# HKUST-Aerial-Robotics/FUEL

Hardware: AMD Instinct MI355X
Metric: plan_cycles_per_sec (higher is better)
Workload: dtype u64 bit-planes / u16 (u32 beyond 255 voxels) exact squared distances / f32 ESDF / f64 log-odds and B-spline

## Files before the change

### fuel_amd/csrc/esdf.hip

```cpp
#include <algorithm>
#include <cmath>
#include <vector>

#include "fuelmi_internal.h"

template <int MODE>
__device__ __forceinline__ u64 src_word(const u64* __restrict__ infl, const u64* __restrict__ unk, long w) {
  if (MODE == 0) return infl[w] | unk[w];
  if (MODE == 1) return infl[w];
  return ~infl[w];
}

template <int MODE>
__device__ __forceinline__ int nearest_src(const u64* __restrict__ infl, const u64* __restrict__ unk,
                                           long linebit, int zlo, int zhi, int z) {
  int best = -1;
  {
    long pos = linebit + z, end = linebit + zhi;
    long w = pos >> 6;
    u64 word = src_word<MODE>(infl, unk, w) & (~0ull << (pos & 63));
    while (true) {
      if (word) {
        long c = (w << 6) + __builtin_ctzll(word);
        if (c <= end) best = (int)(c - pos);
// ... 361 lines not shown
    o.y = o.y >= BIGD ? INF32 : o.y * o.y;
    o.z = o.z >= BIGD ? INF32 : o.z * o.z;
    o.w = o.w >= BIGD ? INF32 : o.w * o.w;
    *reinterpret_cast<uint4*>(row + zi) = o;
  }
}

#define ZY_ROUNDS 2
__device__ __forceinline__ u64 range_mask(int k, int A, int B) {
  const int lo = max(A - 64 * k, 0), hi = min(B - 64 * k, 63);
  return lo <= hi ? bit_range(lo, hi - lo + 1) : 0ull;
}

template <int MODE, bool FAR>
__global__ void __launch_bounds__(512)
k_esdf_zy4(Geo g, Box3 b, const u64* __restrict__ infl, const u64* __restrict__ unk, u32* __restrict__ tmp,
           int ZC, int nzc, int z0a, int near, u32* __restrict__ stat) {
  extern __shared__ __attribute__((aligned(16))) unsigned char smem_raw[];
  u32* tile = reinterpret_cast<u32*>(smem_raw);
  const int xcd = blockIdx.x & 7, slot = blockIdx.x >> 3;
  const int xrel = xcd + 8 * (slot / nzc);
  if (xrel > b.hi[0] - b.lo[0]) return;
  const int x = b.lo[0] + xrel;
  const int zc0 = z0a + (slot % nzc) * ZC;
  const int ylen = b.hi[1] - b.lo[1] + 1;
  const int T = blockDim.x;
  const int zs = max(zc0, b.lo[2]), ze = min(zc0 + ZC - 1, b.hi[2]);
  unsigned char* bm = smem_raw + (size_t)ylen * ZC * 4;
  u32* cm = reinterpret_cast<u32*>(bm + (size_t)((ylen + 7) >> 3) * ZC * 4);
  if (FAR && (int)threadIdx.x < ZC) cm[threadIdx.x] = INF32;
  const u64 inbox_mask = zs <= ze ? bit_range(zs - zc0, ze - zs + 1) : 0ull;
  const bool fastrow = (near >> 8) & 1;
  near &= 0xff;
  if (b.hi[2] - z0a + 1 <= 129 && ylen <= ZY_ROUNDS * T) {
    u64 L[ZY_ROUNDS][3];
#pragma unroll
    for (int r = 0; r < ZY_ROUNDS; ++r) {
      const int yi = threadIdx.x + r * T;
      L[r][0] = L[r][1] = L[r][2] = 0ull;
      if (yi < ylen && zs <= ze) {
        const long linebit = (long)x * g.nyz + (long)(b.lo[1] + yi) * g.nz;
        const long w0 = (linebit + z0a) >> 6, w1 = (linebit + b.hi[2]) >> 6;
        L[r][0] = src_word<MODE>(infl, unk, w0);
        if (w0 + 1 <= w1) L[r][1] = src_word<MODE>(infl, unk, w0 + 1);
        if (w0 + 2 <= w1) L[r][2] = src_word<MODE>(infl, unk, w0 + 2);
      }
    }
#pragma unroll
    for (int r = 0; r < ZY_ROUNDS; ++r) {
      const int yi = threadIdx.x + r * T;
      if (yi >= ylen) break;
      const long linebit = (long)x * g.nyz + (long)(b.lo[1] + yi) * g.nz;
      u64 bits = 0ull;
      int below = -1, above = -1;
      if (zs <= ze) {
        const u64 L0 = L[r][0], L1 = L[r][1], L2 = L[r][2];
        const int p0 = (int)((linebit + z0a) & 63) - z0a;
        const int pc = p0 + zc0, q = pc >> 6, sh = pc & 63;
        const u64 a = q == 0 ? L0 : (q == 1 ? L1 : L2), c = q == 0 ? L1 : (q == 1 ? L2 : 0ull);
        bits = sh ? ((a >> sh) | (c << (64 - sh))) : a;
        bits &= bit_range(zs - zc0, ze - zs + 1);
        if (zs - 1 >= b.lo[2]) {
          const int A = p0 + b.lo[2], B = p0 + zs - 1;
          const u64 m2 = L2 & range_mask(2, A, B), m1 = L1 & range_mask(1, A, B), m0 = L0 & range_mask(0, A, B);
          const int hp = m2 ? 191 - __builtin_clzll(m2) : (m1 ? 127 - __builtin_clzll(m1) : (m0 ? 63 - __builtin_clzll(m0) : -1));
          if (hp >= 0) below = hp - p0;
        }
        if (ze + 1 <= b.hi[2]) {
          const int A = p0 + ze + 1, B = p0 + b.hi[2];
          const u64 m0 = L0 & range_mask(0, A, B), m1 = L1 & range_mask(1, A, B), m2 = L2 & range_mask(2, A, B);
          const int lp = m0 ? __builtin_ctzll(m0) : (m1 ? 64 + __builtin_ctzll(m1) : (m2 ? 128 + __builtin_ctzll(m2) : -1));
          if (lp >= 0) above = lp - p0;
        }
      }
      zy_fill_row(tile + yi * ZC, ZC, bits, below, above, zs, ze, inbox_mask, fastrow);
    }
  } else {
    for (int yi = threadIdx.x; yi < ylen; yi += T) {
      const long linebit = (long)x * g.nyz + (long)(b.lo[1] + yi) * g.nz;
      u64 bits = 0ull;
      int below = -1, above = -1;
      if (zs <= ze) {
        u64 lo = src_word<MODE>(infl, unk, (linebit + zc0) >> 6), hi = src_word<MODE>(infl, unk, ((linebit + zc0) >> 6) + 1);
        int sh = (int)((linebit + zc0) & 63);
        bits = sh ? ((lo >> sh) | (hi << (64 - sh))) : lo;
        bits &= bit_range(zs - zc0, ze - zs + 1);
        below = line_src_down<MODE>(infl, unk, linebit, b.lo[2], zs - 1);
        above = line_src_up<MODE>(infl, unk, linebit, ze + 1, b.hi[2]);
      }
      zy_fill_row(tile + yi * ZC, ZC, bits, below, above, zs, ze, inbox_mask, fastrow);
    }
  }
  __syncthreads();
  if (FAR) {
    build_block_minima(smem_raw, bm, cm, ZC * 4, ZC >> 2, ylen);
    __syncthreads();
  }
  const int G = ZC >> 2;
  const int total = ylen * G;
  const int stride = ZC * 4;
  const int dyi = T / G, dgi = T - dyi * G;
  const bool sampled = stat != nullptr && ((x & 15) == 0 || xrel == 0);
  int n_far = 0;
  const bool z_aligned = (b.lo[2] & 3) == 0 && (b.hi[2] & 3) == 3;
  int yi = threadIdx.x / G, gi = threadIdx.x - yi * G;
  for (int o = threadIdx.x; o < total; o += T) {
    const uint4 bb = scan_line4<FAR>(smem_raw, bm, reinterpret_cast<const unsigned char*>(cm), stride, ylen, yi, 16 * gi, near);
    if (sampled) n_far += __popcll(__ballot(min(min(bb.x, bb.y), min(bb.z, bb.w)) > ESDF_FAR_D * ESDF_FAR_D));
    const int z = zc0 + 4 * gi;
    u32* dst = tmp + (long)x * g.nyz + (long)(b.lo[1] + yi) * g.nz + z;
    if (z_aligned) {
      if (z >= b.lo[2] && z <= b.hi[2]) store16(dst, bb);
    } else if (z >= b.lo[2] && z + 3 <= b.hi[2]) {
      *reinterpret_cast<uint4*>(dst) = bb;
    } else {
      if (z >= b.lo[2] && z <= b.hi[2]) dst[0] = bb.x;
      if (z + 1 >= b.lo[2] && z + 1 <= b.hi[2]) dst[1] = bb.y;
      if (z + 2 >= b.lo[2] && z + 2 <= b.hi[2]) dst[2] = bb.z;
      if (z + 3 >= b.lo[2] && z + 3 <= b.hi[2]) dst[3] = bb.w;
    }
    yi += dyi;
    gi += dgi;
    if (gi >= G) {
      gi -= G;
      ++yi;
    }
  }
  if (sampled && (threadIdx.x & 63) == 0) {
    u32* sg = stat + 2 * ((x >> 4) & (ESDF_NG - 1));
    atomicAdd(sg, (u32)n_far);
    if (threadIdx.x == 0) atomicAdd(sg + 1, (u32)total);
  }
}

#define PK_INF 65025u
typedef unsigned short u16x2_t __attribute__((ext_vector_type(2)));
__device__ __forceinline__ u16x2_t pk_v(u32 v) { return __builtin_bit_cast(u16x2_t, v); }
__device__ __forceinline__ u32 pk_u(u16x2_t v) { return __builtin_bit_cast(u32, v); }
__device__ __forceinline__ u32 pk_min(u32 a, u32 b) { return pk_u(__builtin_elementwise_min(pk_v(a), pk_v(b))); }
__device__ __forceinline__ u32 pk_max(u32 a, u32 b) { return pk_u(__builtin_elementwise_max(pk_v(a), pk_v(b))); }
__device__ __forceinline__ u32 pk_adds(u32 a, u32 b) { return pk_u(__builtin_elementwise_add_sat(pk_v(a), pk_v(b))); }
__device__ __forceinline__ u32 pk_add(u32 a, u32 b) { return pk_u(pk_v(a) + pk_v(b)); }
__device__ __forceinline__ u32 pk_mul(u32 a, u32 b) { return pk_u(pk_v(a) * pk_v(b)); }
__device__ __forceinline__ u32 pk_swap(u32 a) {
  const u16x2_t v = pk_v(a);
  const u16x2_t r = {v.y, v.x};
  return pk_u(r);
}
__device__ __forceinline__ u32 pk_hmax(u32 a) { return max(a & 0xffffu, a >> 16); }
__device__ __forceinline__ u32 pk_hmin(u32 a) { return min(a & 0xffffu, a >> 16); }
__device__ __forceinline__ u32 pk_both(u32 v) { return v | (v << 16); }
__device__ __forceinline__ u32 pk_sat16(u32 v) { return min(v, 0xffffu); }

struct RowSrc {
  u64 bits;
  int below, above;
};
template <int NW>
struct LineBits {
  u64 w[NW];
};
template <int MODE, int NW>
__device__ __forceinline__ LineBits<NW> line_load(const u64* __restrict__ infl, const u64* __restrict__ unk, long linebit,
                                                  int z0a, int zlo, int zhi) {
  const long bit0 = linebit + z0a;
  const long w0 = bit0 >> 6;
  const int sh = (int)(bit0 & 63);
  u64 L[NW + 1];
#pragma unroll
  for (int k = 0; k <= NW; ++k) L[k] = src_word<MODE>(infl, unk, w0 + k);
  LineBits<NW> r;
#pragma unroll
  for (int k = 0; k < NW; ++k) {
    const int lo = max(zlo - z0a - 64 * k, 0), hi = min(zhi - z0a - 64 * k, 63);
    const u64 mask = lo <= hi ? bit_range(lo, hi - lo + 1) : 0ull;
    r.w[k] = (sh ? ((L[k] >> sh) | (L[k + 1] << (64 - sh))) : L[k]) & mask;
  }
  return r;
}
template <int NW>
__device__ __forceinline__ u32 line_bits32(const LineBits<NW>& L, int s) {
  const int k = s >> 6, sh = s & 63;
  u64 lo = 0ull, hi = 0ull;
#pragma unroll
  for (int i = 0; i < NW; ++i) {
    if (i == k) lo = L.w[i];
    if (i == k + 1) hi = L.w[i];
  }
  return (u32)(sh ? ((lo >> sh) | (hi << (64 - sh))) : lo);
}
template <int NW>
__device__ __forceinline__ int line_first_from(const LineBits<NW>& L, int s) {
  int pos = -1;
#pragma unroll
  for (int i = NW - 1; i >= 0; --i) {
    u64 m = L.w[i];
    if (64 * i + 63 < s)
      m = 0ull;
    else if (64 * i < s)
      m &= ~0ull << (s - 64 * i);
    if (m) pos = 64 * i + __builtin_ctzll(m);
  }
  return pos;
}
template <int NW>
__device__ __forceinline__ int line_last_below(const LineBits<NW>& L, int s) {
  int pos = -1;
#pragma unroll
  for (int i = 0; i < NW; ++i) {
    u64 m = L.w[i];
    if (64 * i >= s)
      m = 0ull;
    else if (64 * i + 64 > s)
      m &= (1ull << (s - 64 * i)) - 1ull;
    if (m) pos = 64 * i + 63 - __builtin_clzll(m);
  }
  return pos;
}
template <int NW, bool BELOW>
__device__ __forceinline__ RowSrc row_src_line(const LineBits<NW>& L, int z0a, int zc0, int ZC) {
  RowSrc r;
  const int s = zc0 - z0a;
  r.bits = (u64)(line_bits32<NW>(L, s) & (ZC == 32 ? 0xffffffffu : ((1u << ZC) - 1u)));
  const int up = line_first_from<NW>(L, s + ZC);
  r.above = up >= 0 ? z0a + up : -1;
  r.below = -1;
  if (BELOW) {
    const int dn = line_last_below<NW>(L, s);
    r.below = dn >= 0 ? z0a + dn : -1;
  }
  return r;
}

__device__ __forceinline__ u32 bit_fill(u32 v, int zi) {
  u32 r;
  asm("v_bfe_i32 %0, %1, %2, 1" : "=v"(r) : "v"(v), "s"(zi));
  return r;
}
template <int G>
__device__ __forceinline__ u32 zy_fill_pair(u32* prow, u32 bA, u32 bB, u32 d0, int aboveA, int aboveB, int ze, u32 inbox, bool fast) {
  constexpr int ZC = 4 * G;
  const u32 full = ZC == 32 ? 0xffffffffu : ((1u << (ZC & 31)) - 1u);
  if (fast) {
    const bool all_src = bA == inbox && bB == inbox && inbox != 0u;
    const bool no_src = (bA | bB) == 0u && d0 == 0x00ff00ffu && aboveA < 0 && aboveB < 0;
    if (__ballot(!(all_src | no_src)) == 0ull) {
      const u32 v = all_src ? 0u : pk_both(PK_INF);
      const uint4 o = make_uint4(v, v, v, v);
#pragma unroll
      for (int k = 0; k < G; ++k) *reinterpret_cast<uint4*>(prow + 4 * k) = o;
      if (inbox != full) {
        const u32 ib = inbox | (threadIdx.x & 0u);
        for (int zi = 0; zi < ZC; ++zi) prow[zi] &= bit_fill(ib, zi);
      }
      return all_src ? 0u : 0x00ff00ffu;
    }
  }
  const u32 nA = ~bA, nB = ~bB;
  u32 nm[ZC];
  u32 d = d0;
#pragma unroll
  for (int k = 0; k < G; ++k) {
    u32 f[4];
#pragma unroll
    for (int q = 0; q < 4; ++q) {
      const int zi = 4 * k + q;
      nm[zi] = (bit_fill(nA, zi) & 0xffffu) | (bit_fill(nB, zi) & 0xffff0000u);
      d = pk_add(d, 0x00010001u) & nm[zi];
      f[q] = d;
    }
    *reinterpret_cast<uint4*>(prow + 4 * k) = make_uint4(f[0], f[1], f[2], f[3]);
  }
  const u32 d_end = pk_min(d, 0x00ff00ffu);
  d = (aboveA >= 0 ? (u32)min(aboveA - (ze + 1), 255) : 255u) | ((aboveB >= 0 ? (u32)min(aboveB - (ze + 1), 255) : 255u) << 16);
#pragma unroll
  for (int k = G - 1; k >= 0; --k) {
    const uint4 fw = *reinterpret_cast<const uint4*>(prow + 4 * k);
    const u32 f[4] = {fw.x, fw.y, fw.z, fw.w};
    u32 o[4];
#pragma unroll
    for (int q = 3; q >= 0; --q) {
      d = pk_add(d, 0x00010001u) & nm[4 * k + q];
      const u32 t = pk_min(pk_min(f[q], d), 0x00ff00ffu);
      o[q] = pk_mul(t, t);
    }
    *reinterpret_cast<uint4*>(prow + 4 * k) = make_uint4(o[0], o[1], o[2], o[3]);
  }
  if (inbox != full) {
    const u32 ib = inbox | (threadIdx.x & 0u);
    for (int zi = 0; zi < ZC; ++zi) prow[zi] &= bit_fill(ib, zi);
  }
  return d_end;
}
__device__ __forceinline__ u32 pk_below_d0(const RowSrc& A, const RowSrc& B, int zs) {
  return (A.below >= 0 ? (u32)min(zs - 1 - A.below, 255) : 255u) | ((B.below >= 0 ? (u32)min(zs - 1 - B.below, 255) : 255u) << 16);
}

__device__ __noinline__ u32 pk_slow_col(const u32* tile, int ZC, int ylen, int row, int zcol) {
  u32 best = INF32;
  const int rmax = max(row, ylen - 1 - row);
  for (int r = 0; r <= rmax && (u32)(r * r) < best; ++r) {
    const u32 rr = (u32)(r * r);
    if (row - r >= 0) {
      const int q = row - r;
      const u32 v = (tile[(q >> 1) * ZC + zcol] >> (16 * (q & 1))) & 0xffffu;
      if (v < PK_INF) best = min(best, v + rr);
    }
    if (r && row + r < ylen) {
      const int q = row + r;
      const u32 v = (tile[(q >> 1) * ZC + zcol] >> (16 * (q & 1))) & 0xffffu;
      if (v < PK_INF) best = min(best, v + rr);
    }
  }
  return best;
}

template <int G, bool TILE_SLOW = true>
__device__ __forceinline__ void pk_scan8(const unsigned char* tile_b, int p, int gi, int npair, int ylen, bool any_src,
                                         bool sampled, int& n_far, uint4& ra, uint4& rb) {
  constexpr int ZC = 4 * G;
  constexpr int stride = ZC * 4;
  const u32* tile = reinterpret_cast<const u32*>(tile_b);
    const int col = 16 * gi, base = __mul24(p, stride) + col;
    if (!any_src) {
      ra = rb = make_uint4(INF32, INF32, INF32, INF32);
      if (sampled) n_far += __popcll(__ballot(1));
    } else {
      const uint4 v = lds4(tile_b, base);
      u32 b0 = pk_min(v.x, pk_adds(pk_swap(v.x), 0x00010001u)), b1 = pk_min(v.y, pk_adds(pk_swap(v.y), 0x00010001u));
      u32 b2 = pk_min(v.z, pk_adds(pk_swap(v.z), 0x00010001u)), b3 = pk_min(v.w, pk_adds(pk_swap(v.w), 0x00010001u));
      u32 mx = pk_hmax(pk_max(pk_max(b0, b1), pk_max(b2, b3)));
      const int hi_off = __mul24(npair - 1, stride) + col;
      const int jmax = max(p, npair - 1 - p);
      int od = base, ou = base;
      u32 ro2 = 1u, j8 = 8u;
      for (int j = 1; j <= jmax && ro2 < mx; ++j) {
        od = max(od - stride, col);
        ou = min(ou + stride, hi_off);
        const uint4 pd = lds4(tile_b, od), pu = lds4(tile_b, ou);
        const u32 rn2 = ro2 + j8;
        const u32 re2 = (ro2 + rn2 - 2u) >> 1;
        const u32 ke = pk_both(pk_sat16(re2));
        const u32 k1 = pk_sat16(ro2) | (pk_sat16(rn2) << 16), k2 = pk_sat16(rn2) | (pk_sat16(ro2) << 16);
        b0 = pk_min(b0, pk_min(pk_adds(pk_min(pd.x, pu.x), ke), pk_min(pk_adds(pk_swap(pd.x), k1), pk_adds(pk_swap(pu.x), k2))));
        b1 = pk_min(b1, pk_min(pk_adds(pk_min(pd.y, pu.y), ke), pk_min(pk_adds(pk_swap(pd.y), k1), pk_adds(pk_swap(pu.y), k2))));
        b2 = pk_min(b2, pk_min(pk_adds(pk_min(pd.z, pu.z), ke), pk_min(pk_adds(pk_swap(pd.z), k1), pk_adds(pk_swap(pu.z), k2))));
        b3 = pk_min(b3, pk_min(pk_adds(pk_min(pd.w, pu.w), ke), pk_min(pk_adds(pk_swap(pd.w), k1), pk_adds(pk_swap(pu.w), k2))));
        mx = pk_hmax(pk_max(pk_max(b0, b1), pk_max(b2, b3)));
        ro2 = rn2;
        j8 += 8u;
      }
      if (sampled) n_far += __popcll(__ballot(pk_hmin(pk_min(pk_min(b0, b1), pk_min(b2, b3))) > ESDF_FAR_D * ESDF_FAR_D));
      ra = make_uint4(b0 & 0xffffu, b1 & 0xffffu, b2 & 0xffffu, b3 & 0xffffu);
      rb = make_uint4(b0 >> 16, b1 >> 16, b2 >> 16, b3 >> 16);
      if (TILE_SLOW && mx >= PK_INF) {
        const int zc = 4 * gi, rA = 2 * p, rB = 2 * p + 1;
        if (ra.x >= PK_INF) ra.x = pk_slow_col(tile, ZC, ylen, rA, zc);
        if (ra.y >= PK_INF) ra.y = pk_slow_col(tile, ZC, ylen, rA, zc + 1);
        if (ra.z >= PK_INF) ra.z = pk_slow_col(tile, ZC, ylen, rA, zc + 2);
        if (ra.w >= PK_INF) ra.w = pk_slow_col(tile, ZC, ylen, rA, zc + 3);
        if (rB < ylen) {
          if (rb.x >= PK_INF) rb.x = pk_slow_col(tile, ZC, ylen, rB, zc);
          if (rb.y >= PK_INF) rb.y = pk_slow_col(tile, ZC, ylen, rB, zc + 1);
          if (rb.z >= PK_INF) rb.z = pk_slow_col(tile, ZC, ylen, rB, zc + 2);
          if (rb.w >= PK_INF) rb.w = pk_slow_col(tile, ZC, ylen, rB, zc + 3);
        }
      }
    }
}

__device__ __forceinline__ void forward_stat(u32* stat, volatile u32* h_stat_v) {
  if (stat == nullptr || blockIdx.x != 0) return;
  unsigned long long* h_stat = reinterpret_cast<unsigned long long*>(const_cast<u32*>(h_stat_v));
  const u32 e = stat[2 * ESDF_NG] + 1u;
  const unsigned long long tag = (unsigned long long)(e % 65535u + 1u) << 48;
  for (int g = threadIdx.x; g < ESDF_NG; g += blockDim.x) {
    uint2 p = *reinterpret_cast<const uint2*>(stat + 2 * g);
    if (p.y) {
      *reinterpret_cast<uint2*>(stat + 2 * g) = make_uint2(0u, 0u);
      while (p.y >> 24) p.x >>= 1, p.y >>= 1;
      h_stat[g] = (unsigned long long)p.x | ((unsigned long long)p.y << 24) | tag;
    }
  }
  __syncthreads();
  if (threadIdx.x == 0) stat[2 * ESDF_NG] = e;
}

template <int OUT>
__device__ __forceinline__ void x_store4(float* dst, int z, int zlo, int zhi, uint4 bb, float resf) {
  if (OUT == 0) {
    if ((zlo & 3) == 0 && (zhi & 3) == 3) {
      store16(dst, make_uint4(__float_as_uint(esdf_out(bb.x, resf)), __float_as_uint(esdf_out(bb.y, resf)),
                              __float_as_uint(esdf_out(bb.z, resf)), __float_as_uint(esdf_out(bb.w, resf))));
    } else if (z >= zlo && z + 3 <= zhi) {
      *reinterpret_cast<float4*>(dst) =
          make_float4(esdf_out(bb.x, resf), esdf_out(bb.y, resf), esdf_out(bb.z, resf), esdf_out(bb.w, resf));
    } else {
      if (z >= zlo && z <= zhi) dst[0] = esdf_out(bb.x, resf);
      if (z + 1 >= zlo && z + 1 <= zhi) dst[1] = esdf_out(bb.y, resf);
      if (z + 2 >= zlo && z + 2 <= zhi) dst[2] = esdf_out(bb.z, resf);
      if (z + 3 >= zlo && z + 3 <= zhi) dst[3] = esdf_out(bb.w, resf);
    }
  } else {
    if (z >= zlo && z <= zhi) dst[0] = esdf_merge_neg(dst[0], bb.x, resf);
    if (z + 1 >= zlo && z + 1 <= zhi) dst[1] = esdf_merge_neg(dst[1], bb.y, resf);
    if (z + 2 >= zlo && z + 2 <= zhi) dst[2] = esdf_merge_neg(dst[2], bb.z, resf);
    if (z + 3 >= zlo && z + 3 <= zhi) dst[3] = esdf_merge_neg(dst[3], bb.w, resf);
  }
}

template <int OUT, int SEGS, bool FAR>
__global__ void __launch_bounds__(1024)
k_esdf_x4(Geo g, Box3 b, const u32* __restrict__ tmp, float* __restrict__ dist, int z0a, int zlen_a, int near,
          u32* stat, volatile u32* h_stat) {
  extern __shared__ __attribute__((aligned(16))) unsigned char smem_raw[];
  forward_stat(stat, h_stat);
  uint4* tile = reinterpret_cast<uint4*>(smem_raw);
  const int xlen = b.hi[0] - b.lo[0] + 1;
  const int ylen = b.hi[1] - b.lo[1] + 1;
  const int ncol = ylen * zlen_a;
  const int seg = threadIdx.x & (SEGS - 1);
  const int row0 = threadIdx.x / SEGS;
  const int rows = blockDim.x / SEGS;
  const int col = blockIdx.x * (4 * SEGS) + seg * 4;
  const bool valid = col < ncol;
  const int yy = valid ? col / zlen_a : 0;
  const int z = z0a + (valid ? col - yy * zlen_a : 0);
  const long coloff = (long)(b.lo[1] + yy) * g.nz + z;
  const uint4 inf4 = make_uint4(INF32, INF32, INF32, INF32);
  const float resf = (float)g.res;
  unsigned char* bm = smem_raw + (size_t)xlen * SEGS * 16;
  u32* cm = reinterpret_cast<u32*>(bm + (size_t)((xlen + 7) >> 3) * SEGS * 16);
#pragma unroll 4
  for (int xi = row0; xi < xlen; xi += rows)
    tile[xi * SEGS + seg] = valid ? *reinterpret_cast<const uint4*>(tmp + (long)(b.lo[0] + xi) * g.nyz + coloff) : inf4;
  if (FAR && (int)threadIdx.x < 4 * SEGS) cm[threadIdx.x] = INF32;
  __syncthreads();
  if (FAR) {
    build_block_minima(smem_raw, bm, cm, SEGS * 16, SEGS, xlen);
    __syncthreads();
  }
  if (!valid) return;
  for (int xi = row0; xi < xlen; xi += rows) {
    const uint4 bb = scan_line4<FAR>(smem_raw, bm, reinterpret_cast<const unsigned char*>(cm), SEGS * 16, xlen, xi, 16 * seg, near);
    x_store4<OUT>(dist + (long)(b.lo[0] + xi) * g.nyz + coloff, z, b.lo[2], b.hi[2], bb, resf);
  }
}

#define PK_NOSRC 0xFFFFu
extern "C" __device__ int __ockl_wgred_or_i32(int a);

template <int G>
__device__ __forceinline__ void pk_scan16(const unsigned char* tA, const unsigned char* tB, int p, int gi, int npair, int want,
                                          u32 (&a)[4], u32 (&c)[4]) {
  constexpr int stride = 16 * G;
  const int col = 16 * gi, base = __mul24(p, stride) + col;
  const uint4 vA = lds4(tA, base), vB = lds4(tB, base);
  const u32 one = 0x00010001u;
  a[0] = pk_min(vA.x, pk_adds(pk_swap(vA.x), one)), a[1] = pk_min(vA.y, pk_adds(pk_swap(vA.y), one));
  a[2] = pk_min(vA.z, pk_adds(pk_swap(vA.z), one)), a[3] = pk_min(vA.w, pk_adds(pk_swap(vA.w), one));
  c[0] = pk_min(vB.x, pk_adds(pk_swap(vB.x), one)), c[1] = pk_min(vB.y, pk_adds(pk_swap(vB.y), one));
  c[2] = pk_min(vB.z, pk_adds(pk_swap(vB.z), one)), c[3] = pk_min(vB.w, pk_adds(pk_swap(vB.w), one));
  const u32 mA = (want & 1) ? 0xffffffffu : 0u, mB = (want & 2) ? 0xffffffffu : 0u;
  u32 mx = pk_hmax(pk_max(pk_max(pk_max(a[0], a[1]), pk_max(a[2], a[3])) & mA, pk_max(pk_max(c[0], c[1]), pk_max(c[2], c[3])) & mB));
  const int hi_off = __mul24(npair - 1, stride) + col;
  const int jmax = max(p, npair - 1 - p);
  int od = base, ou = base;
  u32 ro2 = 1u, j8 = 8u;
  for (int j = 1; j <= jmax && ro2 < mx; ++j) {
    od = max(od - stride, col);
    ou = min(ou + stride, hi_off);
    const uint4 dA = lds4(tA, od), uA = lds4(tA, ou), dB = lds4(tB, od), uB = lds4(tB, ou);
    const u32 rn2 = ro2 + j8;
    const u32 re2 = (ro2 + rn2 - 2u) >> 1;
    const u32 ke = pk_both(pk_sat16(re2));
    const u32 k1 = pk_sat16(ro2) | (pk_sat16(rn2) << 16), k2 = pk_sat16(rn2) | (pk_sat16(ro2) << 16);
#define PK16_STEP(B, D, U) B = pk_min(B, pk_min(pk_adds(pk_min(D, U), ke), pk_min(pk_adds(pk_swap(D), k1), pk_adds(pk_swap(U), k2))))
    PK16_STEP(a[0], dA.x, uA.x);
    PK16_STEP(a[1], dA.y, uA.y);
    PK16_STEP(a[2], dA.z, uA.z);
    PK16_STEP(a[3], dA.w, uA.w);
    PK16_STEP(c[0], dB.x, uB.x);
    PK16_STEP(c[1], dB.y, uB.y);
    PK16_STEP(c[2], dB.z, uB.z);
    PK16_STEP(c[3], dB.w, uB.w);
#undef PK16_STEP
    mx = pk_hmax(pk_max(pk_max(pk_max(a[0], a[1]), pk_max(a[2], a[3])) & mA, pk_max(pk_max(c[0], c[1]), pk_max(c[2], c[3])) & mB));
    ro2 = rn2;
    j8 += 8u;
  }
}

__device__ __forceinline__ size_t pk2_index(int tile, int q, int seg, int npx) { return ((size_t)tile * npx + q) * 8 + seg; }

__device__ __forceinline__ u32 pk2_encode(u32 exact, u32* wide_at, bool in_box) {
  if (exact >= INF32) return PK_NOSRC;
  if (exact < PK_INF) return exact;
  if (in_box) *wide_at = exact;
  return PK_INF;
}


template <int MODE, int G, int NW>
__device__ __forceinline__ void zy_pk2_body(const Geo& g, const Box3& b, const u64* __restrict__ infl, const u64* __restrict__ unk,
                                            uint4* __restrict__ tmp16, u32* __restrict__ wide, int z0a, int seg0, int tile0, int tstride, int gsh,
                                            int off, int npx, int q, int fastrow, u32* __restrict__ stat, u32* __restrict__ src_flag, u32 serial,
                                            unsigned long long* stamp, unsigned char* smem_raw) {
  constexpr int ZC = 4 * G;
  const int xA = b.lo[0] + 2 * q, xB = min(xA + 1, b.hi[0]);
  const int zc0 = z0a + 4 * seg0;
  const int ylen = b.hi[1] - b.lo[1] + 1;
  const int npair = (ylen + 1) >> 1;
  const int T = blockDim.x, TH = T >> 1;
  const int half = (int)threadIdx.x >= TH ? 1 : 0;
  const int x = half ? xB : xA;
  unsigned char* tA = smem_raw;
  unsigned char* tB = smem_raw + (size_t)npair * ZC * 4;
  u32* tile = reinterpret_cast<u32*>(half ? tB : tA);
  const int zs = max(zc0, b.lo[2]), ze = min(zc0 + ZC - 1, b.hi[2]);
  const u32 inbox = zs <= ze ? (u32)bit_range(zs - zc0, ze - zs + 1) : 0u;
  bool has_src = false;
  for (int p = (int)threadIdx.x - half * TH; p < npair; p += TH) {
    const int yA = 2 * p, yB = min(2 * p + 1, ylen - 1);
    const long lbA = (long)x * g.nyz + (long)(b.lo[1] + yA) * g.nz;
    const long lbB = (long)x * g.nyz + (long)(b.lo[1] + yB) * g.nz;
    RowSrc A, B;
    A.bits = B.bits = 0ull;
    A.below = A.above = B.below = B.above = -1;
    if (zs <= ze) {
      const LineBits<NW> LA = line_load<MODE, NW>(infl, unk, lbA, z0a, b.lo[2], b.hi[2]);
      const LineBits<NW> LB = line_load<MODE, NW>(infl, unk, lbB, z0a, b.lo[2], b.hi[2]);
      A = row_src_line<NW, true>(LA, z0a, zc0, ZC);
      B = row_src_line<NW, true>(LB, z0a, zc0, ZC);
    }
    has_src |= (A.bits | B.bits) != 0ull || A.below >= 0 || A.above >= 0 || B.below >= 0 || B.above >= 0;
    (void)zy_fill_pair<G>(tile + p * ZC, (u32)A.bits, (u32)B.bits, pk_below_d0(A, B, zs), A.above, B.above, ze, inbox, (fastrow & 1) != 0);
  }
  if (stamp && threadIdx.x == 0) stamp[1] = wall_clock64();
  const int want = __ockl_wgred_or_i32(has_src ? (1 << half) : 0);
  if (stamp && threadIdx.x == 0) stamp[2] = wall_clock64();
  if (want && threadIdx.x == 0) *src_flag = serial;
  const int total = npair * G;
  const bool sampA = stat != nullptr && ((xA & 15) == 0 || q == 0);
  const bool sampB = stat != nullptr && xB != xA && (xB & 15) == 0;
  int n_farA = 0, n_farB = 0;
  for (int o = threadIdx.x; o < total; o += T) {
    const int p = o / G, gi = o - p * G;
    u32 a[4], c[4];
    if (want) {
      pk_scan16<G>(tA, tB, p, gi, npair, want, a, c);
    } else {
      a[0] = a[1] = a[2] = a[3] = c[0] = c[1] = c[2] = c[3] = pk_both(PK_INF);
    }
    if (sampA) n_farA += __popcll(__ballot(!(want & 1) || pk_hmin(pk_min(pk_min(a[0], a[1]), pk_min(a[2], a[3]))) > ESDF_FAR_D * ESDF_FAR_D));
    if (sampB) n_farB += __popcll(__ballot(!(want & 2) || pk_hmin(pk_min(pk_min(c[0], c[1]), pk_min(c[2], c[3]))) > ESDF_FAR_D * ESDF_FAR_D));
    uint4 r0, r1;
    const u32 mxa = pk_hmax(pk_max(pk_max(a[0], a[1]), pk_max(a[2], a[3]))), mxc = pk_hmax(pk_max(pk_max(c[0], c[1]), pk_max(c[2], c[3])));
    if (max(mxa, mxc) < PK_INF) {
      r0 = make_uint4(__builtin_amdgcn_perm(c[0], a[0], 0x05040100u), __builtin_amdgcn_perm(c[1], a[1], 0x05040100u),
                      __builtin_amdgcn_perm(c[2], a[2], 0x05040100u), __builtin_amdgcn_perm(c[3], a[3], 0x05040100u));
      r1 = make_uint4(__builtin_amdgcn_perm(c[0], a[0], 0x07060302u), __builtin_amdgcn_perm(c[1], a[1], 0x07060302u),
                      __builtin_amdgcn_perm(c[2], a[2], 0x07060302u), __builtin_amdgcn_perm(c[3], a[3], 0x07060302u));
    } else {
      const int zc = 4 * gi, rA = 2 * p, rB = min(2 * p + 1, ylen - 1);
      u32 w0[4], w1[4];
#pragma unroll
      for (int k = 0; k < 4; ++k) {
        const int z = zc0 + zc + k;
        const bool in_box = z >= b.lo[2] && z <= b.hi[2];
        u32 e[4];
        e[0] = a[k] & 0xffffu, e[1] = a[k] >> 16, e[2] = c[k] & 0xffffu, e[3] = c[k] >> 16;
#pragma unroll
        for (int v = 0; v < 4; ++v) {
          const bool slabB = v >= 2;
          const int row = (v & 1) ? rB : rA;
          if (!((want >> (slabB ? 1 : 0)) & 1))
            e[v] = in_box ? PK_NOSRC : 0u;
          else if (e[v] >= PK_INF) {
            const u32 ex = pk_slow_col(reinterpret_cast<const u32*>(slabB ? tB : tA), ZC, ylen, row, zc + k);
            u32* wat = wide + (long)(slabB ? xB : xA) * g.nyz + (long)(b.lo[1] + row) * g.nz + z;
            e[v] = pk2_encode(ex, wat, in_box);
          }
        }
        w0[k] = e[0] | (e[2] << 16), w1[k] = e[1] | (e[3] << 16);
      }
      r0 = make_uint4(w0[0], w0[1], w0[2], w0[3]);
      r1 = make_uint4(w1[0], w1[1], w1[2], w1[3]);
    }
    {
      const int y = 2 * p, ry1 = (8 >> gsh) - 1;
      store16(tmp16 + pk2_index(tile0 + (y >> (3 - gsh)) * tstride, q, ((y & ry1) << gsh) + off + gi, npx), r0);
    }
    if (2 * p + 1 < ylen) {
      const int y = 2 * p + 1, ry1 = (8 >> gsh) - 1;
      store16(tmp16 + pk2_index(tile0 + (y >> (3 - gsh)) * tstride, q, ((y & ry1) << gsh) + off + gi, npx), r1);
    }
  }
  if (stamp && threadIdx.x == 0) stamp[3] = wall_clock64();
  if ((sampA | sampB) && (threadIdx.x & 63) == 0) {
    if (sampA) {
      u32* sg = stat + 2 * ((xA >> 4) & (ESDF_NG - 1));
      atomicAdd(sg, (u32)n_farA);
      if (threadIdx.x == 0) atomicAdd(sg + 1, (u32)total);
    }
    if (sampB) {
      u32* sg = stat + 2 * ((xB >> 4) & (ESDF_NG - 1));
      atomicAdd(sg, (u32)n_farB);
      if (threadIdx.x == 0) atomicAdd(sg + 1, (u32)total);
    }
  }
}

template <int MODE, int GMAX, int NW>
__global__ void __launch_bounds__(1024)
k_esdf_zy_pk2(Geo g, Box3 b, const u64* __restrict__ infl, const u64* __restrict__ unk, uint4* __restrict__ tmp16,
              u32* __restrict__ wide, Pk2ZChunks ch, int z0a, int npx, int fastrow, u32* __restrict__ stat,
              u32* __restrict__ src_flag, u32 serial, unsigned long long* __restrict__ dbg) {
  extern __shared__ __attribute__((aligned(16))) unsigned char smem_raw[];
  const int nzc = ch.n;
  const int xcd = blockIdx.x & 7, slot = blockIdx.x >> 3;
  const int q = xcd + 8 * (slot / nzc);
  if (q >= npx) return;
  unsigned long long* stamp = dbg ? dbg + 8 * (size_t)blockIdx.x : nullptr;
  if (stamp && threadIdx.x == 0) stamp[0] = wall_clock64();
  const int c = slot % nzc;
  const int seg0 = ch.seg0[c], tile0 = ch.tile0[c], tstride = ch.tstride[c], gsh = ch.gsh[c], off = ch.off[c];
#define PK2_BODY(GG) zy_pk2_body<MODE, GG, NW>(g, b, infl, unk, tmp16, wide, z0a, seg0, tile0, tstride, gsh, off, npx, q, fastrow, stat, src_flag, serial, stamp, smem_raw)
  switch (ch.g[c]) {
    case 8:
      if constexpr (GMAX >= 8) PK2_BODY(8);
      break;
    case 4:
      if constexpr (GMAX >= 4) PK2_BODY(4);
      break;
    case 2: PK2_BODY(2); break;
    default: PK2_BODY(1); break;
  }
#undef PK2_BODY
}

__device__ __noinline__ u32 x_slow_col16(const u32* tile, int c, const u32* __restrict__ wide_col, long row_stride, int xlen, int row) {
  u32 best = INF32;
  const int rmax = max(row, xlen - 1 - row);
  for (int r = 0; r <= rmax && (u32)__mul24(r, r) < best; ++r) {
    const u32 rr = (u32)__mul24(r, r);
#pragma unroll
    for (int s = 0; s < 2; ++s) {
      const int qrow = s ? row + r : row - r;
      if (qrow < 0 || qrow >= xlen || (s && !r)) continue;
      u32 v = (tile[(qrow >> 1) * 32 + c] >> (16 * (qrow & 1))) & 0xffffu;
      if (v == PK_NOSRC) continue;
      if (v >= PK_INF) v = wide_col[(long)qrow * row_stride];
      best = min(best, v + rr);
    }
  }
  return best;
}

template <int OUT>
__global__ void __launch_bounds__(512)
k_esdf_x_pk2(Geo g, Box3 b, const uint4* __restrict__ tmp16, const u32* __restrict__ wide, float* __restrict__ dist, Pk2Chunks ch,
             int z0a, int full8, u32* stat, volatile u32* h_stat, const u32* __restrict__ src_flag, u32 serial,
             unsigned long long* __restrict__ dbg) {
  constexpr int SEGS = 8;
  extern __shared__ __attribute__((aligned(16))) unsigned char smem_raw[];
  forward_stat(stat, h_stat);
  uint4* tile = reinterpret_cast<uint4*>(smem_raw);
  const int xlen = b.hi[0] - b.lo[0] + 1;
  const int ylen = b.hi[1] - b.lo[1] + 1;
  const int npx = (xlen + 1) >> 1;
  const int T = blockDim.x;
  const int total = npx * SEGS;
  const float resf = (float)g.res;
  unsigned long long* stamp = dbg ? dbg + 8 * (size_t)blockIdx.x : nullptr;
  if (stamp && threadIdx.x == 0) stamp[0] = wall_clock64();
  int gw = 8, gsh = 3, y0, seg0, t;
  if ((int)blockIdx.x < full8) {
    const int xcd = blockIdx.x & 7, slot = blockIdx.x >> 3;
    y0 = xcd + 8 * (slot / ch.n8);
    if (y0 >= ylen) return;
    const int c8 = slot % ch.n8;
    seg0 = 8 * c8;
    t = y0 * ch.n8 + c8;
  } else {
    t = (int)blockIdx.x - full8 + ylen * ch.n8;
    int c = ch.n8;
    while (c + 1 < ch.n && t >= ch.tile0[c + 1]) ++c;
    gw = ch.g[c], gsh = gw == 4 ? 2 : (gw == 2 ? 1 : 0);
    y0 = (t - ch.tile0[c]) * (8 >> gsh);
    seg0 = ch.seg0[c];
  }
  const bool any_src = *src_flag == serial;
  if (any_src) {
    const uint4* src = tmp16 + pk2_index(t, 0, 0, npx);
#pragma unroll 4
    for (int o = threadIdx.x; o < total; o += T) tile[o] = src[o];
  }
  if (stamp && threadIdx.x == 0) stamp[1] = wall_clock64();
  __syncthreads();
  if (stamp && threadIdx.x == 0) stamp[2] = wall_clock64();
  int n_far = 0;
  for (int o = threadIdx.x; o < total; o += T) {
    const int p = o >> 3, seg = o & 7;
    const int yy = y0 + (seg >> gsh);
    if (yy >= ylen) continue;
    uint4 ra, rb;
    pk_scan8<SEGS, false>(smem_raw, p, seg, npx, xlen, any_src, false, n_far, ra, rb);
    const int z = z0a + 4 * (seg0 + (seg & (gw - 1)));
    const long coloff = (long)(b.lo[1] + yy) * g.nz + z;
    if (any_src && max(max4(ra.x, ra.y, ra.z, ra.w), max4(rb.x, rb.y, rb.z, rb.w)) >= PK_INF) {
      u32* pa = &ra.x;
      u32* pb = &rb.x;
      const u32* wc = wide + (long)b.lo[0] * g.nyz + coloff;
      for (int k = 0; k < 4; ++k) {
        if (pa[k] >= PK_INF) pa[k] = x_slow_col16(reinterpret_cast<const u32*>(smem_raw), 4 * seg + k, wc + k, g.nyz, xlen, 2 * p);
        if (2 * p + 1 < xlen && pb[k] >= PK_INF)
          pb[k] = x_slow_col16(reinterpret_cast<const u32*>(smem_raw), 4 * seg + k, wc + k, g.nyz, xlen, 2 * p + 1);
      }
    }
    float* dst = dist + (long)(b.lo[0] + 2 * p) * g.nyz + coloff;
    x_store4<OUT>(dst, z, b.lo[2], b.hi[2], ra, resf);
    if (2 * p + 1 < xlen) x_store4<OUT>(dst + g.nyz, z, b.lo[2], b.hi[2], rb, resf);
  }
  if (stamp && threadIdx.x == 0) stamp[3] = wall_clock64();
}


static hipError_t lds_attr_once(const void* fn, int bytes) {
  static std::mutex mu;
  static std::vector<std::pair<const void*, int>> done;
  int dev = 0;
  (void)hipGetDevice(&dev);
  std::lock_guard<std::mutex> lk(mu);
  for (const auto& d : done)
    if (d.first == fn && d.second == dev) return hipSuccess;
  const hipError_t e = hipFuncSetAttribute(fn, hipFuncAttributeMaxDynamicSharedMemorySize, bytes);
  if (e == hipSuccess) done.push_back({fn, dev});
  return e;
}

static int pass_timing_report(fuelmi_map* m, unsigned long long* dbg, int grid, const char* what) {
  HIPCHK(hipStreamSynchronize(m->stream));
  std::vector<unsigned long long> d((size_t)grid * 8);
  HIPCHK(hipMemcpy(d.data(), dbg, d.size() * sizeof(unsigned long long), hipMemcpyDeviceToHost));
  HIPCHK(hipFree(dbg));
  unsigned long long t0 = ~0ull, t1 = 0;
  double ph[3] = {0, 0, 0}, life = 0;
  int n = 0;
  for (int w = 0; w < grid; ++w) {
    const unsigned long long* r = &d[(size_t)w * 8];
    if (!r[0] || !r[3]) continue;
    t0 = std::min(t0, r[0]), t1 = std::max(t1, r[3]);
    ph[0] += (double)(r[1] - r[0]), ph[1] += (double)(r[2] - r[1]), ph[2] += (double)(r[3] - r[2]), life += (double)(r[3] - r[0]);
    ++n;
  }
  int alive = 0, early = 0;
  const unsigned long long mid = t0 + (t1 - t0) / 2;
  for (int w = 0; w < grid; ++w) {
    const unsigned long long* r = &d[(size_t)w * 8];
    if (!r[0] || !r[3]) continue;
    if (r[0] <= mid && r[3] >= mid) ++alive;
    if (r[0] - t0 < 100) ++early;
  }
  std::vector<double> st, en;
  for (int w = 0; w < grid; ++w) {
    const unsigned long long* r = &d[(size_t)w * 8];
    if (!r[0] || !r[3]) continue;
    st.push_back((double)(r[0] - t0) / 100.0), en.push_back((double)(r[3] - t0) / 100.0);
  }
  std::sort(st.begin(), st.end());
  std::sort(en.begin(), en.end());
  int peak = 0;
  {
    size_t i = 0, j = 0;
    int cur = 0;
    while (i < st.size()) {
      if (st[i] <= en[j]) ++cur, ++i, peak = std::max(peak, cur);
      else --cur, ++j;
    }
  }
  {
    std::vector<std::pair<double, int>> lv;
    for (int w = 0; w < grid; ++w) {
      const unsigned long long* r = &d[(size_t)w * 8];
      if (!r[0] || !r[3]) continue;
      lv.push_back({(double)(r[3] - r[0]) / 100.0, w});
    }
    std::sort(lv.begin(), lv.end());
    const size_t k0 = lv.size() - std::max<size_t>(1, lv.size() / 10);
    double f = 0, bb = 0, sc = 0, lf = 0;
    for (size_t k = k0; k < lv.size(); ++k) {
      const unsigned long long* r = &d[(size_t)lv[k].second * 8];
      f += (double)(r[1] - r[0]), bb += (double)(r[2] - r[1]), sc += (double)(r[3] - r[2]), lf += lv[k].first;
    }
    const double nn = (double)(lv.size() - k0) * 100.0;
    std::fprintf(stderr, "[slowest tenth: fill %.2f barrier %.2f scan %.2f life %.2f us; slowest blocks:", f / nn, bb / nn, sc / nn, lf * 100.0 / nn);
    for (size_t k = lv.size() - std::min<size_t>(8, lv.size()); k < lv.size(); ++k) std::fprintf(stderr, " %d(%.1f)", lv[k].second, lv[k].first);
    std::fprintf(stderr, "]\n");
  }
  auto pct = [](const std::vector<double>& v, double f) { return v.empty() ? 0.0 : v[std::min(v.size() - 1, (size_t)(f * (double)v.size()))]; };
  std::fprintf(stderr, "[%s: %d workgroups, span %.2f us; per workgroup: fill %.2f barrier %.2f scan %.2f life %.2f us; "
               "alive at mid-span %d (peak %d), started in the first us %d; starts 25/50/75/100 %%: %.1f %.1f %.1f %.1f us, ends 25/50/75: %.1f %.1f %.1f\n",
               what, n, (double)(t1 - t0) / 100.0, ph[0] / n / 100.0,
               ph[1] / n / 100.0, ph[2] / n / 100.0, life / n / 100.0, alive, peak, early, pct(st, 0.25), pct(st, 0.5), pct(st, 0.75),
               pct(st, 1.0), pct(en, 0.25), pct(en, 0.5), pct(en, 0.75));
  return FUELMI_OK;
}


static bool pk2_chunks(int ylen, int nseg, int gz_max, Pk2Chunks* xs, Pk2ZChunks* zs) {
  *xs = Pk2Chunks{};
  *zs = Pk2ZChunks{};
  const int n8 = nseg >> 3;
  int n = 0, nz = 0, seg = 0, tile = ylen * n8;
  auto add_z = [&](int seg_lo, int gw, int gsh, int tile0, int tstride) {
    const int gz = std::min(gw, gz_max);
    for (int o = 0; o < gw; o += gz) {
      if (nz == PK2_MAXZCH) return false;
      zs->seg0[nz] = (short)(seg_lo + o), zs->g[nz] = (signed char)gz, zs->gsh[nz] = (signed char)gsh, zs->off[nz] = (signed char)o;
      zs->tile0[nz] = tile0, zs->tstride[nz] = tstride;
      ++nz;
    }
    return true;
  };
  for (int c = 0; c < n8; ++c, ++n, seg += 8) {
    if (n == PK2_MAXCH) return false;
    xs->seg0[n] = (short)seg, xs->g[n] = 8, xs->tile0[n] = 0;
    if (!add_z(seg, 8, 3, c, n8)) return false;
  }
  xs->n8 = n8;
  while (seg < nseg) {
    int gw = 4;
    while (gw > nseg - seg) gw >>= 1;
    const int gsh = gw == 4 ? 2 : (gw == 2 ? 1 : 0);
    if (n == PK2_MAXCH) return false;
    xs->seg0[n] = (short)seg, xs->g[n] = (short)gw, xs->tile0[n] = tile;
    if (!add_z(seg, gw, gsh, tile, 1)) return false;
    tile += (ylen + 8 / gw - 1) / (8 / gw);
    seg += gw;
    ++n;
  }
  xs->n = n;
  zs->n = nz;
  for (int k = n; k <= PK2_MAXCH; ++k) xs->tile0[k] = tile;
  for (int k = n; k < PK2_MAXCH; ++k) xs->g[k] = 1;
  if (n8 == n) xs->tile0[n8] = tile;
  return true;
}

size_t esdf_handover_bytes(int nx, int ny, int nz) {
  if (nz % 4 != 0) return 0;
  const size_t ntiles = ((size_t)ny * (size_t)((nz + 7) / 4 + 1) + 7) / 8 + PK2_MAXCH + 1;
  return ntiles * (size_t)(((nx + 1) / 2 + 63) / 64) * 64 * 128;
}

struct EsdfLaunch {
  int kernel = 0, targ[3] = {0, 0, 0};
  int grid = 0, block = 0, lds = 0;
  int ZC = 0, nzc = 0, z0a = 0;
  int aux = 0;
};
struct EsdfPlan {
  int n = 0;
  int family = 0;
  EsdfLaunch l[4];
  Pk2Chunks ch;
  Pk2ZChunks zch;
};

static int esdf_plan(const int dims[3], const Box3& b, int family, bool optimistic, bool signed_dist, size_t handover,
                     EsdfPlan* p) {
  *p = EsdfPlan{};
  const int xlen = b.hi[0] - b.lo[0] + 1, ylen = b.hi[1] - b.lo[1] + 1, zlen = b.hi[2] - b.lo[2] + 1;
  const int z0a = b.lo[2] & ~3, zlen_a = (b.hi[2] | 3) - z0a + 1;
  const int npx = (xlen + 1) >> 1, npair = (ylen + 1) >> 1;
  const bool z4 = dims[2] % 4 == 0;
  const int g_max = (size_t)npair * 4 * 32 > 52 * 1024 ? 2 : 4;
  const size_t pk2_lds = (size_t)npair * g_max * 32;
  const bool pk2 = z4 && zlen <= 255 && handover > 0 && (size_t)npx * 128 <= 150 * 1024 && pk2_lds <= 160 * 1024 - 64 &&
                   pk2_chunks(ylen, zlen_a >> 2, g_max, &p->ch, &p->zch) &&
                   (size_t)p->ch.tile0[p->ch.n] * npx * 128 <= handover;
  const bool vec4 = z4 && (size_t)xlen * 64 <= 150 * 1024;

  auto pass = [&](int fam, int mode, EsdfLaunch* L, int* ran) {
    const int out = mode == 2;
    EsdfLaunch& zy = L[0];
    EsdfLaunch& x = L[1];
    if (fam == FUELMI_ESDF_PLAIN && pk2) {
      zy = {FUELMI_ESDF_K_ZY_PK2, {mode, g_max, zlen_a > 128 ? 4 : 2}, ((npx + 7) / 8) * 8 * p->zch.n,
            2 * std::min(256, std::max(64, ((npair / 2 + 63) / 64) * 64)), (int)pk2_lds, 0, p->zch.n, z0a, npx};
      const int x_lds = npx * 8 * 16;
      const int full8 = ((ylen + 7) / 8) * 8 * p->ch.n8;
      x = {FUELMI_ESDF_K_X_PK2, {out, 0, 0}, full8 + (p->ch.tile0[p->ch.n] - ylen * p->ch.n8), x_lds > 32 * 1024 ? 512 : 256,
           x_lds, 0, p->ch.n, z0a, full8};
      *ran = FUELMI_ESDF_PLAIN;
      return FUELMI_OK;
    }
    const bool far = fam == FUELMI_ESDF_FAR;
    *ran = far ? FUELMI_ESDF_FAR : FUELMI_ESDF_PLAIN32;
    if (vec4) {
      const int budget = std::min(std::max(32 * 1024, ylen * 4 * 20), 80 * 1024);
      int zc_max = std::max(4, (budget / (4 * ylen)) & ~3);
      zc_max = std::min(zc_max, std::min(zlen_a, 64));
      int nzc = (zlen_a + zc_max - 1) / zc_max;
      const int ZC = (((zlen_a + nzc - 1) / nzc) + 3) & ~3;
      nzc = (zlen_a + ZC - 1) / ZC;
      auto zy_lds = [&](bool f) { return (size_t)(f ? ylen + ((ylen + 7) >> 3) + 1 : ylen) * ZC * sizeof(u32); };
      const bool zy_far = far && zy_lds(true) <= 160 * 1024;
      if (zy_lds(zy_far) > 160 * 1024) {
        fuelmi_set_error("ESDF y-line of %d voxels does not fit the LDS tile", ylen);
        return FUELMI_ELIMIT;
      }
      zy = {FUELMI_ESDF_K_ZY4, {mode, zy_far, 0}, ((xlen + 7) / 8) * 8 * nzc, 512, (int)zy_lds(zy_far), ZC, nzc, z0a, 0};
      const int segs = (size_t)xlen * 128 > 150 * 1024 ? 4 : 8;
      auto x_lds = [&](bool f) { return (size_t)(f ? xlen + ((xlen + 7) >> 3) + 1 : xlen) * segs * 4 * sizeof(u32); };
      const bool x_far = far && x_lds(true) <= 160 * 1024;
      x = {FUELMI_ESDF_K_X4, {out, segs, x_far}, (ylen * zlen_a + 4 * segs - 1) / (4 * segs), 1024, (int)x_lds(x_far), 0, 0,
           z0a, zlen_a};
      return FUELMI_OK;
    }
    const int zc_max = std::min(std::min(std::max(1, (16 * 1024) / (2 * ylen)), zlen), 256);
    const int nzc = (zlen + zc_max - 1) / zc_max;
// ... 190 lines not shown
```

Before: 11160.

## Flatten ESDF z-fill row loop and compute nearest-source keys with packed bit scans

Replaces the per-half thread split with one flat loop over both x-columns' row pairs, so each thread handles whichever pair comes next and the halves share the block evenly. The fast path now tests for an empty line across the whole loaded window before the search and skips the above/below nearest-source search entirely for uniform waves. Nearest-source search is rewritten as a template-specialized sweep over 32-bit halves with v_ffbl/v_ffbh and min-reduction, replacing branchy ctz/clz loops. It also adds optional debug counters for how many waves took the shortcut, with a stderr report.

```diff
diff --git a/fuel_amd/csrc/esdf.hip b/fuel_amd/csrc/esdf.hip
--- a/fuel_amd/csrc/esdf.hip
+++ b/fuel_amd/csrc/esdf.hip
@@ -537,10 +537,6 @@
 __device__ __forceinline__ u32 pk_both(u32 v) { return v | (v << 16); }
 __device__ __forceinline__ u32 pk_sat16(u32 v) { return min(v, 0xffffu); }
 
-struct RowSrc {
-  u64 bits;
-  int below, above;
-};
 template <int NW>
 struct LineBits {
   u64 w[NW];
@@ -575,46 +571,11 @@
   return (u32)(sh ? ((lo >> sh) | (hi << (64 - sh))) : lo);
 }
 template <int NW>
-__device__ __forceinline__ int line_first_from(const LineBits<NW>& L, int s) {
-  int pos = -1;
+__device__ __forceinline__ u64 line_any(const LineBits<NW>& L) {
+  u64 v = L.w[0];
 #pragma unroll
-  for (int i = NW - 1; i >= 0; --i) {
-    u64 m = L.w[i];
-    if (64 * i + 63 < s)
-      m = 0ull;
-    else if (64 * i < s)
-      m &= ~0ull << (s - 64 * i);
-    if (m) pos = 64 * i + __builtin_ctzll(m);
-  }
-  return pos;
-}
-template <int NW>
-__device__ __forceinline__ int line_last_below(const LineBits<NW>& L, int s) {
-  int pos = -1;
-#pragma unroll
-  for (int i = 0; i < NW; ++i) {
-    u64 m = L.w[i];
-    if (64 * i >= s)
-      m = 0ull;
-    else if (64 * i + 64 > s)
-      m &= (1ull << (s - 64 * i)) - 1ull;
-    if (m) pos = 64 * i + 63 - __builtin_clzll(m);
-  }
-  return pos;
-}
-template <int NW, bool BELOW>
-__device__ __forceinline__ RowSrc row_src_line(const LineBits<NW>& L, int z0a, int zc0, int ZC) {
-  RowSrc r;
-  const int s = zc0 - z0a;
-  r.bits = (u64)(line_bits32<NW>(L, s) & (ZC == 32 ? 0xffffffffu : ((1u << ZC) - 1u)));
-  const int up = line_first_from<NW>(L, s + ZC);
-  r.above = up >= 0 ? z0a + up : -1;
-  r.below = -1;
-  if (BELOW) {
-    const int dn = line_last_below<NW>(L, s);
-    r.below = dn >= 0 ? z0a + dn : -1;
-  }
-  return r;
+  for (int i = 1; i < NW; ++i) v |= L.w[i];
+  return v;
 }
 
 __device__ __forceinline__ u32 bit_fill(u32 v, int zi) {
@@ -623,24 +584,9 @@
   return r;
 }
 template <int G>
-__device__ __forceinline__ u32 zy_fill_pair(u32* prow, u32 bA, u32 bB, u32 d0, int aboveA, int aboveB, int ze, u32 inbox, bool fast) {
+__device__ __forceinline__ u32 zy_fill_pair(u32* prow, u32 bA, u32 bB, u32 d0, u32 up0, u32 inbox) {
   constexpr int ZC = 4 * G;
   const u32 full = ZC == 32 ? 0xffffffffu : ((1u << (ZC & 31)) - 1u);
-  if (fast) {
-    const bool all_src = bA == inbox && bB == inbox && inbox != 0u;
-    const bool no_src = (bA | bB) == 0u && d0 == 0x00ff00ffu && aboveA < 0 && aboveB < 0;
-    if (__ballot(!(all_src | no_src)) == 0ull) {
-      const u32 v = all_src ? 0u : pk_both(PK_INF);
-      const uint4 o = make_uint4(v, v, v, v);
-#pragma unroll
-      for (int k = 0; k < G; ++k) *reinterpret_cast<uint4*>(prow + 4 * k) = o;
-      if (inbox != full) {
-        const u32 ib = inbox | (threadIdx.x & 0u);
-        for (int zi = 0; zi < ZC; ++zi) prow[zi] &= bit_fill(ib, zi);
-      }
-      return all_src ? 0u : 0x00ff00ffu;
-    }
-  }
   const u32 nA = ~bA, nB = ~bB;
   u32 nm[ZC];
   u32 d = d0;
@@ -657,7 +603,7 @@
     *reinterpret_cast<uint4*>(prow + 4 * k) = make_uint4(f[0], f[1], f[2], f[3]);
   }
   const u32 d_end = pk_min(d, 0x00ff00ffu);
-  d = (aboveA >= 0 ? (u32)min(aboveA - (ze + 1), 255) : 255u) | ((aboveB >= 0 ? (u32)min(aboveB - (ze + 1), 255) : 255u) << 16);
+  d = up0;
 #pragma unroll
   for (int k = G - 1; k >= 0; --k) {
     const uint4 fw = *reinterpret_cast<const uint4*>(prow + 4 * k);
@@ -677,8 +623,72 @@
   }
   return d_end;
 }
-__device__ __forceinline__ u32 pk_below_d0(const RowSrc& A, const RowSrc& B, int zs) {
-  return (A.below >= 0 ? (u32)min(zs - 1 - A.below, 255) : 255u) | ((B.below >= 0 ? (u32)min(zs - 1 - B.below, 255) : 255u) << 16);
+template <int G>
+__device__ __forceinline__ void zy_fill_const(u32* prow, u32 v, u32 inbox) {
+  constexpr int ZC = 4 * G;
+  const u32 full = ZC == 32 ? 0xffffffffu : ((1u << (ZC & 31)) - 1u);
+  const uint4 o = make_uint4(v, v, v, v);
+#pragma unroll
+  for (int k = 0; k < G; ++k) *reinterpret_cast<uint4*>(prow + 4 * k) = o;
+  if (inbox != full) {
+    const u32 ib = inbox | (threadIdx.x & 0u);
+    for (int zi = 0; zi < ZC; ++zi) prow[zi] &= bit_fill(ib, zi);
+  }
+}
+
+__device__ __forceinline__ u32 ffbl32(u32 v) {
+  u32 r;
+  asm("v_ffbl_b32 %0, %1" : "=v"(r) : "v"(v));
+  return r;
+}
+__device__ __forceinline__ u32 ffbh32(u32 v) {
+  u32 r;
+  asm("v_ffbh_u32 %0, %1" : "=v"(r) : "v"(v));
+  return r;
+}
+struct PairKeys {
+  u32 dnA, dnB;
+  u32 upA, upB;
+};
+template <int NW, int C>
+__device__ __forceinline__ PairKeys line_pair_search_at(const LineBits<NW>& LA, const LineBits<NW>& LB, u32 mlo, u32 mhi) {
+  PairKeys k;
+  k.dnA = k.dnB = k.upA = k.upB = 0xffffffffu;
+#pragma unroll
+  for (int j = 0; j < 2 * NW; ++j) {
+    const u32 a = (u32)(LA.w[j >> 1] >> (32 * (j & 1))), c = (u32)(LB.w[j >> 1] >> (32 * (j & 1)));
+    if (j <= C) {
+      const u32 hi = 32u * (u32)(2 * NW - 1 - j);
+      k.dnA = min(k.dnA, ffbh32(j == C ? a & mlo : a) | hi);
+      k.dnB = min(k.dnB, ffbh32(j == C ? c & mlo : c) | hi);
+    }
+    if (j >= C) {
+      k.upA = min(k.upA, ffbl32(j == C ? a & mhi : a) | (u32)(32 * j));
+      k.upB = min(k.upB, ffbl32(j == C ? c & mhi : c) | (u32)(32 * j));
+    }
+  }
+  return k;
+}
+template <int NW>
+__device__ __forceinline__ PairKeys line_pair_search(const LineBits<NW>& LA, const LineBits<NW>& LB, int s, int ZC) {
+  const int lo = s & 31, hi = lo + ZC;
+  const u32 mlo = (1u << lo) - 1u, mhi = hi >= 32 ? 0u : 0xffffffffu << hi;
+  switch (s >> 5) {
+    case 0: return line_pair_search_at<NW, 0>(LA, LB, mlo, mhi);
+    case 1: return line_pair_search_at<NW, 1>(LA, LB, mlo, mhi);
+    case 2: return line_pair_search_at<NW, 2>(LA, LB, mlo, mhi);
+    default: break;
+  }
+  if constexpr (NW > 2) {
+    switch (s >> 5) {
+      case 3: return line_pair_search_at<NW, 3>(LA, LB, mlo, mhi);
+      case 4: return line_pair_search_at<NW, 4>(LA, LB, mlo, mhi);
+      case 5: return line_pair_search_at<NW, 5>(LA, LB, mlo, mhi);
+      case 6: return line_pair_search_at<NW, 6>(LA, LB, mlo, mhi);
+      default: break;
+    }
+  }
+  return line_pair_search_at<NW, 2 * NW - 1>(LA, LB, mlo, mhi);
 }
 
 __device__ __noinline__ u32 pk_slow_col(const u32* tile, int ZC, int ylen, int row, int zcol) {
@@ -896,33 +906,53 @@
   const int zc0 = z0a + 4 * seg0;
   const int ylen = b.hi[1] - b.lo[1] + 1;
   const int npair = (ylen + 1) >> 1;
-  const int T = blockDim.x, TH = T >> 1;
-  const int half = (int)threadIdx.x >= TH ? 1 : 0;
-  const int x = half ? xB : xA;
+  const int T = blockDim.x;
   unsigned char* tA = smem_raw;
   unsigned char* tB = smem_raw + (size_t)npair * ZC * 4;
-  u32* tile = reinterpret_cast<u32*>(half ? tB : tA);
   const int zs = max(zc0, b.lo[2]), ze = min(zc0 + ZC - 1, b.hi[2]);
   const u32 inbox = zs <= ze ? (u32)bit_range(zs - zc0, ze - zs + 1) : 0u;
-  bool has_src = false;
-  for (int p = (int)threadIdx.x - half * TH; p < npair; p += TH) {
+  int src_bits = 0;
+  for (int i = (int)threadIdx.x; i < 2 * npair; i += T) {
+    const int half = i >= npair ? 1 : 0;
+    const int p = i - (half ? npair : 0);
+    const int x = half ? xB : xA;
+    u32* tile = reinterpret_cast<u32*>(half ? tB : tA);
+    u32* prow = tile + p * ZC;
     const int yA = 2 * p, yB = min(2 * p + 1, ylen - 1);
     const long lbA = (long)x * g.nyz + (long)(b.lo[1] + yA) * g.nz;
     const long lbB = (long)x * g.nyz + (long)(b.lo[1] + yB) * g.nz;
-    RowSrc A, B;
-    A.bits = B.bits = 0ull;
-    A.below = A.above = B.below = B.above = -1;
-    if (zs <= ze) {
-      const LineBits<NW> LA = line_load<MODE, NW>(infl, unk, lbA, z0a, b.lo[2], b.hi[2]);
-      const LineBits<NW> LB = line_load<MODE, NW>(infl, unk, lbB, z0a, b.lo[2], b.hi[2]);
-      A = row_src_line<NW, true>(LA, z0a, zc0, ZC);
-      B = row_src_line<NW, true>(LB, z0a, zc0, ZC);
-    }
-    has_src |= (A.bits | B.bits) != 0ull || A.below >= 0 || A.above >= 0 || B.below >= 0 || B.above >= 0;
-    (void)zy_fill_pair<G>(tile + p * ZC, (u32)A.bits, (u32)B.bits, pk_below_d0(A, B, zs), A.above, B.above, ze, inbox, (fastrow & 1) != 0);
+    u32 bA = 0u, bB = 0u, d0 = 0x00ff00ffu, up0 = 0x00ff00ffu;
+    if (zs > ze) {
+      if (fastrow & 1)
+        zy_fill_const<G>(prow, pk_both(PK_INF), inbox);
+      else
+        (void)zy_fill_pair<G>(prow, bA, bB, d0, up0, inbox);
+      continue;
+    }
+    const LineBits<NW> LA = line_load<MODE, NW>(infl, unk, lbA, z0a, b.lo[2], b.hi[2]);
+    const LineBits<NW> LB = line_load<MODE, NW>(infl, unk, lbB, z0a, b.lo[2], b.hi[2]);
+    const int s = zc0 - z0a;
+    const u32 cmask = ZC == 32 ? 0xffffffffu : ((1u << ZC) - 1u);
+    bA = line_bits32<NW>(LA, s) & cmask;
+    bB = line_bits32<NW>(LB, s) & cmask;
+    const bool empty = (line_any<NW>(LA) | line_any<NW>(LB)) == 0ull;
+    const bool all_src = bA == inbox && bB == inbox;
+    if (!empty) src_bits |= 1 << half;
+    const bool tally = stamp != nullptr && (threadIdx.x & 63) == 0;
+    if (tally) atomicAdd(&stamp[4], 1ull);
+    if ((fastrow & 1) && __ballot(!(all_src | empty)) == 0ull) {
+      if (tally) atomicAdd(&stamp[5], 1ull);
+      zy_fill_const<G>(prow, all_src ? 0u : pk_both(PK_INF), inbox);
+      continue;
+    }
+    const PairKeys k = line_pair_search<NW>(LA, LB, s, ZC);
+    const u32 dn_off = (u32)(zs - z0a - 64 * NW), up_off = (u32)(z0a - ze - 1);
+    d0 = min(k.dnA + dn_off, 255u) | (min(k.dnB + dn_off, 255u) << 16);
+    up0 = min(k.upA + up_off, 255u) | (min(k.upB + up_off, 255u) << 16);
+    (void)zy_fill_pair<G>(prow, bA, bB, d0, up0, inbox);
   }
   if (stamp && threadIdx.x == 0) stamp[1] = wall_clock64();
-  const int want = __ockl_wgred_or_i32(has_src ? (1 << half) : 0);
+  const int want = __ockl_wgred_or_i32(src_bits);
   if (stamp && threadIdx.x == 0) stamp[2] = wall_clock64();
   if (want && threadIdx.x == 0) *src_flag = serial;
   const int total = npair * G;
@@ -1132,9 +1162,11 @@
   unsigned long long t0 = ~0ull, t1 = 0;
   double ph[3] = {0, 0, 0}, life = 0;
   int n = 0;
+  unsigned long long trips = 0, shortcut = 0;
   for (int w = 0; w < grid; ++w) {
     const unsigned long long* r = &d[(size_t)w * 8];
     if (!r[0] || !r[3]) continue;
+    trips += r[4], shortcut += r[5];
     t0 = std::min(t0, r[0]), t1 = std::max(t1, r[3]);
     ph[0] += (double)(r[1] - r[0]), ph[1] += (double)(r[2] - r[1]), ph[2] += (double)(r[3] - r[2]), life += (double)(r[3] - r[0]);
     ++n;
@@ -1153,6 +1185,8 @@
     if (!r[0] || !r[3]) continue;
     st.push_back((double)(r[0] - t0) / 100.0), en.push_back((double)(r[3] - t0) / 100.0);
   }
+  if (trips)
+    std::fprintf(stderr, "[fill: %llu wave-trips, %llu without a sweep (%.1f %%)]\n", trips, shortcut, 100.0 * (double)shortcut / (double)trips);
   std::sort(st.begin(), st.end());
   std::sort(en.begin(), en.end());
   int peak = 0;
```

Measured after the change: 10960. 1.8% lower.
